# mahyarnajibi/SNIPER

Measured on AMD Instinct MI355X. Metric: train chips/sec (512x512, R101), higher is better.
Workload: dtype f16; 1 GPU; ResNet-101 Faster-RCNN SNIPER 3-scale, batch 20 x 512x512 fp16 per GPU (BASELINE configs[1]); step = GPU anchor labelling + fwd + bwd + grad all-reduce + SGD on HBM-resident chips (epoch chip generation / box assignment and image decode+resize are outside the step); f16 MFMA operands, f32 accumulation / losses / master weights; chips_per_gpu=20, global_batch=20, parallelism=dp1

## Files before the change

include/sniper_hip.h:

```cpp
#ifndef SNIPER_HIP_H
#define SNIPER_HIP_H

#include <stddef.h>
#include <stdint.h>

#ifdef __cplusplus
extern "C" {
#endif

typedef void *sn_stream_t;

enum { SN_OK = 0, SN_ERR_ARG = 1, SN_ERR_HIP = 2, SN_ERR_WORKSPACE = 3, SN_ERR_UNSUPPORTED = 4 };

int sn_version(void);
const char *sn_last_error(void);
int sn_debug_option(const char *name, int value);

int sn_iou_f64(const double *d_boxes, int N, const double *d_query, int K, double *d_out, int mode, sn_stream_t stream);

int sn_chips_num_candidates(int width, int height, int chipsize, int stride);
size_t sn_chips_workspace_bytes(int total_cand, int max_boxes_per_unit);
int sn_chips_generate_batch(const float *d_boxes, const int32_t *d_box_off, const int32_t *d_meta, const int32_t *d_perm,
                            const int32_t *d_cand_off, int U, int max_boxes_per_unit, void *d_mask_ws, float *d_out_chips,
                            int32_t *d_out_ids, int32_t *d_out_count, sn_stream_t stream);
// ... 55 lines not shown
                           int Cout, int out_pix_stride, int KH, int KW, int stride, int pad, int dil, int relu, void *ws,
                           size_t ws_bytes, sn_stream_t stream);
int sn_conv_fwd_dual_ok(int N, int H, int W, int Cin, int in_pix_stride, int Cout, int out_pix_stride, int res_pix_stride, int KH,
                        int KW, int stride, int pad, int dil, int y2_pix_stride);
int sn_conv_fwd_dual(const void *x, const void *w, const float *bias, const void *residual, void *y, int N, int H, int W, int Cin,
                     int in_pix_stride, int Cout, int out_pix_stride, int res_pix_stride, int KH, int KW, int stride, int pad, int dil,
                     int relu, void *y2, int y2_pix_stride, const float *y2_scale, const float *y2_shift, int y2_relu, void *ws,
                     size_t ws_bytes, sn_stream_t stream);
int sn_conv_tune(int cfg);

int sn_conv_fwd_stats_blocks(int N, int H, int W, int Cin, int in_pix_stride, int Cout, int out_pix_stride, int res_pix_stride,
                             int KH, int KW, int stride, int pad, int dil);
int sn_conv_fwd_stats(const void *x, const void *w, const float *bias, const void *residual, void *y, int N, int H, int W, int Cin,
                      int in_pix_stride, int Cout, int out_pix_stride, int res_pix_stride, int KH, int KW, int stride, int pad,
                      int dil, int relu, float *stats, sn_stream_t stream);
int sn_conv_stem_fwd(const void *xp, const void *w, const float *bias, void *y, int N, int Hp, int Wp, int Ho, int Wo, int Cout,
                     int out_pix_stride, int KH, int KWP, int stride, int relu, int out_f32, sn_stream_t stream);
size_t sn_conv_stem_wgrad_workspace_bytes(int N, int Ho, int Wo, int Cout, int KH, int KWP);
int sn_conv_stem_wgrad(const void *dy, const void *xp, float *dw, int N, int Hp, int Wp, int Ho, int Wo, int Cout, int dy_pix_stride,
                       int KH, int KWP, int stride, void *ws, size_t ws_bytes, sn_stream_t stream);
int sn_conv_dgrad(const void *dy, const void *wt, const void *accumulate, void *dx, int N, int H, int W, int Cin,
                  int dx_pix_stride, int Cout, int dy_pix_stride, int acc_pix_stride, int KH, int KW, int stride, int pad, int dil,
                  int out_f32, sn_stream_t stream);
int sn_conv_dgrad_by_class(int on);
int sn_conv_dgrad_bn_blocks(int N, int H, int W, int Cin, int dx_pix_stride, int Cout, int dy_pix_stride, int acc_pix_stride, int KH,
                            int KW, int stride, int pad, int dil);
int sn_conv_dgrad_bn(const void *dy, const void *wt, const void *accumulate, void *dx, int N, int H, int W, int Cin, int dx_pix_stride,
                     int Cout, int dy_pix_stride, int acc_pix_stride, int KH, int KW, int stride, int pad, int dil, const void *bn_x,
                     int bn_x_pix_stride, const float *bn_scale, const float *bn_shift, const float *bn_mean, int bn_act,
                     float *partials, sn_stream_t stream);
// ... 285 lines not shown
```

sniper_amd/csrc/conv.hip:

```cpp
#include <algorithm>
#include <atomic>

#include "conv_common.h"

#include <stdlib.h>

__device__ __forceinline__ int swz(int row, int chunk) { return chunk ^ ((0x78 >> (2 * ((row >> 2) & 3))) & 3); }

template <int BM, int BN, bool DGRAD>
__global__ __launch_bounds__(256) void conv_igemm_kernel(const ConvParams p) {
  constexpr int BK = 32;
  constexpr int WM = BM / 2, WN = BN / 2;
  constexpr int MI = WM / 16, NI = WN / 16;
  constexpr int AR = BM / 64, BR = BN / 64;
  __shared__ __attribute__((aligned(16))) half_t sA[2][BM * BK];
  __shared__ __attribute__((aligned(16))) half_t sB[2][BN * BK];

  const int tid = threadIdx.x, lane = tid & 63, wave = tid >> 6;
  const int wm = wave >> 1, wn = wave & 1;
  const int m0 = blockIdx.x * BM, n0 = blockIdx.y * BN;
  const int chunk = tid & 3, lrow = tid >> 2;

  int a_base[AR], a_h[AR], a_w[AR];
  bool a_ok[AR];
// ... 414 lines not shown
}

SN_EXPORT int sn_conv_fwd_stats(const void *x, const void *w, const float *bias, const void *residual, void *y, int N, int H, int W,
                                int Cin, int in_pix_stride, int Cout, int out_pix_stride, int res_pix_stride, int KH, int KW,
                                int stride, int pad, int dil, int relu, float *stats, sn_stream_t stream) {
  ConvParams p;
  conv_fwd_params(p, x, w, bias, residual, y, N, H, W, Cin, in_pix_stride, Cout, out_pix_stride, res_pix_stride, KH, KW, stride, pad,
                  dil, relu, 0);
  if (int rc = conv_check(p, "sn_conv_fwd_stats")) return rc;
  SN_REQUIRE(stats && Cout % 4 == 0 && out_pix_stride % 4 == 0 && (!residual || res_pix_stride % 4 == 0),
             "sn_conv_fwd_stats: statistics need 8-byte aligned output rows (query sn_conv_fwd_stats_blocks)");
  p.stats = stats;
  return conv_launch<false>(p, sn_stream(stream));
}

SN_EXPORT int sn_conv_stem_fwd(const void *xp, const void *w, const float *bias, void *y, int N, int Hp, int Wp, int Ho, int Wo,
                               int Cout, int out_pix_stride, int KH, int KWP, int stride, int relu, int out_f32,
                               sn_stream_t stream) {
  ConvParams p;
  p.x = (const half_t *)xp; p.w = (const half_t *)w; p.y = y; p.bias = bias; p.res = nullptr;
  p.N = N; p.H = Hp; p.W = Wp; p.Cin = 4 * KWP; p.in_ps = 4;
  p.Ho = Ho; p.Wo = Wo; p.Nout = Cout; p.out_ps = out_pix_stride; p.res_ps = 0;
  p.KH = KH; p.KW = 1; p.stride = stride; p.pad = 0; p.dil = 1;
  p.M = N * Ho * Wo; p.relu = relu; p.out_f32 = out_f32;
  SN_REQUIRE((Ho - 1) * stride + KH <= Hp && (Wo - 1) * stride + KWP <= Wp, "sn_conv_stem_fwd: padded input too small");
  SN_REQUIRE(stride % 2 == 0 && Wp % 2 == 0 && KWP % 2 == 0, "sn_conv_stem_fwd: 16-byte alignment needs even stride/pitch");
  if (int rc = conv_check(p, "sn_conv_stem_fwd")) return rc;
  return conv_launch<false>(p, sn_stream(stream));
}

// ... 375 lines not shown
```

sniper_amd/csrc/conv_common.h:

```cpp
#pragma once
#include <atomic>
#include "common.h"

struct ConvParams {
  const half_t *x;
  const half_t *w;
  void *y;
  const float *bias;
  const half_t *res;
  int N, H, W;
  int Cin, in_ps;
  int Ho, Wo;
  int Nout, out_ps, res_ps;
  int KH, KW, stride, pad, dil;
  int M;
  int relu, out_f32;
  unsigned x_bytes, w_bytes;
  const half_t *bn_x = nullptr;
  const float *bn_scale = nullptr, *bn_shift = nullptr, *bn_mean = nullptr;
  int bn_x_ps = 0, bn_act = 0;
  unsigned fda_mul = 1, fda_sh = 0, fdb_mul = 1, fdb_sh = 0;
  int rows_img = 1, row_len = 1;
  int cls = 0, cls_mc = 0;
  int ksplit = 1, ksplit_grid = 0;
  long ksplit_stride = 0;
  unsigned long long *trace = nullptr;
  half_t *out2 = nullptr;
  const float *o2_scale = nullptr, *o2_shift = nullptr;
  int out2_ps = 0, o2_relu = 0;
  int tiles_per_wg = 1;
  float *stats = nullptr;
};


static inline void conv_fastdiv_fill(ConvParams &p) {
  p.rows_img = p.cls ? (p.Ho / 2) * (p.Wo / 2) : p.Ho * p.Wo;
  p.row_len = p.cls ? p.Wo / 2 : p.Wo;
  const SnDiv a = sn_div_make((unsigned)p.rows_img), b = sn_div_make((unsigned)p.row_len);
  p.fda_mul = a.mul; p.fda_sh = a.sh;
  p.fdb_mul = b.mul; p.fdb_sh = b.sh;
}

typedef __attribute__((address_space(3))) void *lds_ptr_t;
typedef short short4v __attribute__((vector_size(8)));

__device__ __forceinline__ void dma16(__amdgpu_buffer_rsrc_t rsrc, half_t *dst, unsigned voff) {
// ... 13 lines not shown

struct ConvDmaConfig { int bm, bn, threads, stages, lds_bytes; };
constexpr int kConvPersistWgs = 512;
static inline int conv_persist_tiles_per_wg(int M, int Nout, int bm, int bn) {
  if (M % bm || Nout % bn) return 0;
  const long mt = M / bm, nt = Nout / bn, tiles = mt * nt;
  if (mt % 8 || tiles < 2 * kConvPersistWgs || tiles % kConvPersistWgs) return 0;
  return (int)(tiles / kConvPersistWgs);
}
constexpr int kConvDmaConfigs = 26;
ConvDmaConfig conv_dma_config(int cfg);
int conv_dma_launch(const ConvParams &p, bool dgrad, int cfg, hipStream_t s);
void conv_dma_set_trace(unsigned long long *buf);
int conv_dma_ragged_cfg(int cfg, bool dgrad);
int conv_dma_ragged_launch(const ConvParams &p, bool dgrad, int cfg, hipStream_t s);

struct WgradParams {
  const half_t *dy;
  const half_t *x;
  float *dw;
  int N, H, W, Ho, Wo, Cin, Cout, dy_ps, x_ps;
  int KH, KW, stride, pad, dil;
  int units_per_split;
  float *slab;
  size_t slab_stride;
  int gx, gy, gz, per_xcd;
};

__device__ __forceinline__ bool wgrad_block(const WgradParams &p, int &bx, int &by, int &bz) {
  const int b = blockIdx.x;
// ... 38 lines not shown
```

sniper_amd/csrc/conv_dma.hip:

```cpp
#include "conv_dma_kernel.h"

ConvDmaConfig conv_dma_config(int cfg) { return (cfg >= 1 && cfg <= kConvDmaConfigs) ? kCfg[cfg] : kCfg[0]; }

template <bool DGRAD>
static int launch_cfg(const ConvParams &p, int cfg, hipStream_t s) {
  switch (cfg) {
    case 4: launch_config<DGRAD, 4>(p, s); break;
    case 5: launch_config<DGRAD, 5>(p, s); break;
    case 6: launch_config<DGRAD, 6>(p, s); break;
    case 7: launch_config<DGRAD, 7>(p, s); break;
    case 14: launch_config<DGRAD, 14>(p, s); break;
    case 16: launch_config<DGRAD, 16>(p, s); break;
    case 18: launch_config<DGRAD, 18>(p, s); break;
    case 24: launch_config<DGRAD, 24>(p, s); break;
    case 26: launch_config<DGRAD, 26>(p, s); break;
    default: SN_REQUIRE(false, "conv_dma_launch: unknown configuration %d", cfg);
  }
  SN_CHECK_LAUNCH();
  return SN_OK;
}

static std::atomic<unsigned long long *> g_conv_trace{nullptr};
void conv_dma_set_trace(unsigned long long *buf) { g_conv_trace.store(buf, std::memory_order_relaxed); }

int conv_dma_launch(const ConvParams &p, bool dgrad, int cfg, hipStream_t s) {
  ConvParams q = p;
  q.trace = g_conv_trace.load(std::memory_order_relaxed);
  if (p.Cin % 64 != 0) return conv_dma_ragged_launch(q, dgrad, cfg, s);
  return dgrad ? launch_cfg<true>(q, cfg, s) : launch_cfg<false>(q, cfg, s);
}
```

sniper_amd/csrc/conv_dma_body.h:

```cpp
  constexpr int NW = WMW * WNW, T = 64 * (NW + (PS ? 4 : 0)), BK = 64;
  static_assert(!PERSIST || (!PS && S == 2), "the persistent tile loop is written for the two-stage unspecialised pipeline");
  static_assert(!PERSIST || !RAGGED, "the persistent tile loop walks whole 64-channel steps");
  constexpr int NL = PS ? 4 : NW;
  constexpr int WTM = BM / WMW, WTN = BN / WNW;
  constexpr int MI = WTM / 16, NI = WTN / 16;
  constexpr int PA = BM / 8, PB = BN / 8;
  constexpr int AGW = (PA + NL - 1) / NL, BGW = (PB + NL - 1) / NL;
  constexpr int L = AGW + BGW;
  constexpr int STAGE = (BM + BN) * BK;
  constexpr bool kPingPong = NW == 8 && S >= 3;
  static_assert(BM % 8 == 0 && BN % 8 == 0 && WTM % 16 == 0 && WTN % 16 == 0, "tile / wave shape");
  static_assert(PA >= NL * (AGW - 1) + 1 && PB >= NL * (BGW - 1) + 1 && (AGW == 1 ? PA >= NL : true) && (BGW == 1 ? PB >= NL : true),
                "a wave's repeated piece must exist");
  static_assert((S - 1) * L < 64, "vmcnt is a 6-bit counter");
  constexpr int RED = PERSIST ? WMW * 2 * BN * 2 : 0;
  constexpr bool kBnLds = PERSIST && DGRAD;
  constexpr int COEF = kBnLds ? 3 * 512 : 0;
  static_assert(!kBnLds || BN <= 128, "one LDS-DMA piece carries 128 coefficients");
  __shared__ __attribute__((aligned(1024))) half_t lds[S * STAGE + RED + COEF];

  constexpr bool kSplitOk = !PERSIST && !DGRAD && BM * BN <= 160 * 128;
  int kz = 0;
  int lin = blockIdx.x;
  if (kSplitOk && p.ksplit > 1) {
    kz = lin / p.ksplit_grid;
    lin -= kz * p.ksplit_grid;
  }
  auto tile_of = [&](int l, int &mt_, int &nt_) {
    const int xcd = l & 7, j = l >> 3;
    nt_ = j % ntiles;
    mt_ = (j / ntiles) * 8 + xcd;
  };
  int nt, mt;
  tile_of(lin, mt, nt);
// ... 41 lines not shown

  int a_base[AGW], a_h[AGW], a_w[AGW];
  bool a_ok[AGW];
  int a_grp[AGW], b_grp[BGW];
#pragma unroll
  for (int i = 0; i < AGW; ++i) a_grp[i] = (lw + NL * i < PA) ? lw + NL * i : lw + NL * (i - 1);
#pragma unroll
  for (int i = 0; i < BGW; ++i) b_grp[i] = (lw + NL * i < PB) ? lw + NL * i : lw + NL * (i - 1);
  unsigned a_voff[AGW];
  auto gather_rows = [&](int gm0) {
    if constexpr (PERSIST) {
#pragma unroll
      for (int i = 0; i < AGW; ++i) a_voff[i] = (unsigned)(gm0 + 8 * a_grp[i] + lrow) * ((unsigned)p.in_ps * 2u) + (unsigned)gchunk * 16u;
      return;
    }
#pragma unroll
    for (int i = 0; i < AGW; ++i) {
      const int m = gm0 + 8 * a_grp[i] + lrow;
      a_ok[i] = m < Mrows;
      int img, oy, ox;
      row_decompose(a_ok[i] ? m : 0, img, oy, ox);
      a_base[i] = img * p.H * p.W;
      if (DGRAD) { a_h[i] = oy + p.pad; a_w[i] = ox + p.pad; }
      else { a_h[i] = oy * p.stride - p.pad; a_w[i] = ox * p.stride - p.pad; }
    }
  };
  gather_rows(m0);
  const int taps = p.KH * p.KW;
  const int kpt = RAGGED ? (p.Cin + BK - 1) / BK : p.Cin / BK;
  const bool tail_in = !RAGGED || gchunk * 8 < p.Cin - (kpt - 1) * BK;
// ... 17 lines not shown
      const int r = 8 * b_grp[i] + lrow;
      const int n = gn0 + (r & ~31) + ((r & 15) >> 2) * 8 + ((r >> 4) & 1) * 4 + (r & 3);
      w_voff[i] = n < p.Nout ? (unsigned)n * wrow_bytes + (unsigned)gchunk * 16u : kOob;
      if constexpr (RAGGED) w_voff_l[i] = tail_in ? w_voff[i] : kOob;
    }
  };
  gather_cols(n0);
  int g_kh = kh0, g_kw = kw0, g_kc = 0;
  if (kSplitOk && t_begin > 0) {
    const int tap = t_begin / kpt;
    g_kc = t_begin - tap * kpt;
    g_kh = tap / p.KW;
    g_kw = tap - g_kh * p.KW;
  }
  auto tap_setup = [&]() {
    if constexpr (PERSIST) return;
#pragma unroll
    for (int i = 0; i < AGW; ++i) {
      int sy, sx;
      bool ok = a_ok[i];
      if (DGRAD) {
        const int ty = a_h[i] - g_kh * p.dil, tx = a_w[i] - g_kw * p.dil;
        if (p.stride == 1) { sy = ty; sx = tx; }
        else if (p.stride == 2) { sy = ty >> 1; sx = tx >> 1; ok = ok && !((ty | tx) & 1); }
        else { sy = ty / p.stride; sx = tx / p.stride; ok = ok && (sy * p.stride == ty) && (sx * p.stride == tx); }
        ok = ok && ty >= 0 && tx >= 0 && sy < p.H && sx < p.W;
      } else {
        sy = a_h[i] + g_kh * p.dil; sx = a_w[i] + g_kw * p.dil;
        ok = ok && (unsigned)sy < (unsigned)p.H && (unsigned)sx < (unsigned)p.W;
      }
      a_voff[i] = ok ? (unsigned)(a_base[i] + sy * p.W + sx) * in_ps_bytes + (unsigned)gchunk * 16u : kOob;
// ... 12 lines not shown
#pragma unroll
        for (int i = 0; i < AGW; ++i) dma16(rx, sa + a_grp[i] * 512, av[i]);
#pragma unroll
        for (int i = 0; i < BGW; ++i) dma16(rw, sb + b_grp[i] * 512, wv[i]);
      };
      if (g_kc == kpt - 1) pieces(a_voff_l, w_voff_l);
      else pieces(a_voff, w_voff);
    } else {
#pragma unroll
    for (int i = 0; i < AGW; ++i)
      dma16(rx, sa + a_grp[i] * 512, a_voff[i]);
#pragma unroll
    for (int i = 0; i < BGW; ++i)
      dma16(rw, sb + b_grp[i] * 512, w_voff[i]);
    }
    if constexpr (PERSIST) {
      ++g_kc;
    } else if (++g_kc == kpt) {
      g_kc = 0;
      g_kw += kstep;
      if (g_kw >= p.KW) { g_kw = kw0; g_kh += kstep; }
      tap_setup();
    }
  };

  auto fetch_seek = [&](int l, int step) {
    int fmt, fnt;
    tile_of(l, fmt, fnt);
    gather_rows(fmt * BM);
    gather_cols(fnt * BN);
    g_kc = step;
// ... 55 lines not shown
    } else {
      const int m = row_pixel(mr < Mrows ? mr : 0);
      return (mr < Mrows && n < p.Nout) ? *reinterpret_cast<const half8 *>(pre_src + (size_t)m * pre_ps + n) : half8{0, 0, 0, 0, 0, 0, 0, 0};
    }
  };
  auto pre_load_tile = [&](int pm0, int pn0) {
#pragma unroll
    for (int i = 0; i < MI; ++i)
#pragma unroll
      for (int jp = 0; jp < NP; ++jp) rpre[i][jp] = pre_load(pm0, pn0, i, jp);
  };
  if constexpr (kPre) if ((pre_res || pre_bnx) && !producer) pre_load_tile(m0, n0);

  if constexpr (PS) {
    if (producer) {
#pragma unroll
      for (int s = 0; s < S - 1; ++s)
        if (s < nk) issue(s);
      int nxt = S - 1;
      for (int t = 0; t < nk; ++t) {
        const int young = min(S - 2, nk - 1 - t);
        if (S > 3 && young >= 2) wait_vmcnt<(S > 3 ? 2 : 0) * L>();
        else if (S > 2 && young == 1) wait_vmcnt<(S > 2 ? 1 : 0) * L>();
        else wait_vmcnt<0>();
        __builtin_amdgcn_s_barrier();
        if (t + S - 1 < nk) issue(nxt);
        nxt = nxt + 1 == S ? 0 : nxt + 1;
      }
    } else {
      half8 fa0[MI], fb0[NI], fa1[MI], fb1[NI];
      auto read = [&](int buf, int ks, half8 (&fa)[MI], half8 (&fb)[NI]) {
        const half_t *const base = lds + buf * STAGE;
        const int co = (sw ^ (ks * 4)) * 8;
#pragma unroll
        for (int i = 0; i < MI; ++i) fa[i] = *reinterpret_cast<const half8 *>(base + a_rd + i * 16 * BK + co);
#pragma unroll
        for (int jn = 0; jn < NI; ++jn) fb[jn] = *reinterpret_cast<const half8 *>(base + b_rd + jn * 16 * BK + co);
      };
      auto mma = [&](const half8 (&fa)[MI], const half8 (&fb)[NI]) {
// ... 3 lines not shown
          for (int jn = 0; jn < NI; ++jn) acc[i][jn] = __builtin_amdgcn_mfma_f32_16x16x32_f16(fb[jn], fa[i], acc[i][jn], 0, 0, 0);
      };
      auto interleave = [&]() {
#pragma unroll
        for (int k = 0; k < MI + NI; ++k) {
          __builtin_amdgcn_sched_group_barrier(0x008, 2, 0);
          __builtin_amdgcn_sched_group_barrier(0x100, 1, 0);
        }
        __builtin_amdgcn_sched_group_barrier(0x008, MI * NI - 2 * (MI + NI) > 0 ? MI * NI - 2 * (MI + NI) : 0, 0);
        __builtin_amdgcn_sched_barrier(0);
      };
      auto step_barrier = [&]() {
        asm volatile("s_waitcnt lgkmcnt(0)" ::: "memory");
        __builtin_amdgcn_s_barrier();
      };
      if (nk > 0) {
        step_barrier();
        stamp(1);
        read(0, 0, fa0, fb0);
        __builtin_amdgcn_sched_barrier(0);
      }
      int cur = 0, nxt = 1;
      for (int t = 0; t + 1 < nk; ++t) {
        mma(fa0, fb0);
        read(cur, 1, fa1, fb1);
        interleave();
        step_barrier();
        __builtin_amdgcn_sched_barrier(0);
        mma(fa1, fb1);
        read(nxt, 0, fa0, fb0);
// ... 350 lines not shown
```

sniper_amd/csrc/conv_dma_kernel.h:

```cpp
#pragma once
#include "conv_common.h"
#include <type_traits>

template <int CTRL>
__device__ __forceinline__ float dpp_add(float v) {
  return v + __builtin_bit_cast(float, __builtin_amdgcn_update_dpp(0, __builtin_bit_cast(int, v), CTRL, 0xF, 0xF, false));
}
__device__ __forceinline__ float row16_sum(float v) {
  v = dpp_add<0xB1>(v);
  v = dpp_add<0x4E>(v);
  v = dpp_add<0x141>(v);
  return dpp_add<0x140>(v);
}

__device__ __forceinline__ half8 load16_untracked(const half_t *ptr) {
  floatx4 v;
  asm volatile("global_load_dwordx4 %0, %1, off" : "=v"(v) : "v"(ptr) : "memory");
  return __builtin_bit_cast(half8, v);
}
__device__ __forceinline__ floatx4 lds_read16_untracked(const void *ptr) {
  floatx4 v;
  const unsigned a = (unsigned)(unsigned long)(lds_ptr_t)const_cast<void *>(ptr);
  asm volatile("ds_read_b128 %0, %1" : "=v"(v) : "v"(a) : "memory");
  return v;
}
__device__ __forceinline__ void tie(floatx4 &v) { asm volatile("" : "+v"(v)); }
__device__ __forceinline__ void tie(half8 &x) {
  floatx4 v = __builtin_bit_cast(floatx4, x);
  asm volatile("" : "+v"(v));
  x = __builtin_bit_cast(half8, v);
}

template <bool DGRAD, int BM, int BN, int WMW, int WNW, int S, int MINW, bool PS = false, bool PERSIST = false>
__global__ __launch_bounds__(64 * (WMW * WNW + (PS ? 4 : 0)), MINW) void conv_dma_kernel(const ConvParams p, int mtiles, int ntiles) {
  constexpr bool RAGGED = false;
#include "conv_dma_body.h"
}
template <bool DGRAD, int BM, int BN, int WMW, int WNW, int S, int MINW, bool PS = false, bool PERSIST = false>
__global__ __launch_bounds__(64 * (WMW * WNW + (PS ? 4 : 0)), MINW) void conv_dma_ragged_kernel(const ConvParams p, int mtiles, int ntiles) {
  constexpr bool RAGGED = true;
#include "conv_dma_body.h"
}

template <bool DGRAD, int BM, int BN, int WMW, int WNW, int S, int MINW, bool PS = false, bool PERSIST = false, bool RAGGED = false>
static void launch_one(const ConvParams &p, hipStream_t s) {
  const int mtiles = (DGRAD && !PS && p.cls && BM * BN <= 160 * 128) ? 4 * sn_div_up(p.cls_mc, BM) : sn_div_up(p.M, BM), ntiles = sn_div_up(p.Nout, BN);
  const int base = sn_div_up(mtiles, 8) * 8 * ntiles;
  ConvParams q = p;
  q.ksplit_grid = base;
  if constexpr (PERSIST) {
    q.tiles_per_wg = conv_persist_tiles_per_wg(p.M, p.Nout, BM, BN);
    q.ksplit = 1;
    hipLaunchKernelGGL((conv_dma_kernel<DGRAD, BM, BN, WMW, WNW, S, MINW, PS, true>), dim3((unsigned)(base / q.tiles_per_wg)),
                       dim3(64 * WMW * WNW), 0, s, q, mtiles, ntiles);
  } else {
// ... 48 lines not shown
```

sniper_amd/csrc/nn_ops.hip:

```cpp
#include "common.h"
#include "softmax_grad.h"
#include <algorithm>

__global__ __launch_bounds__(256) void pack_stem_kernel(const float *__restrict__ x, half_t *__restrict__ out, int N, int C,
                                                        int H, int W, int Hp, int Wp, int pad_t, int pad_l,
                                                        const float *__restrict__ scale, const float *__restrict__ shift) {
  const long total = (long)N * Hp * Wp;
  for (long i = (long)blockIdx.x * blockDim.x + threadIdx.x; i < total; i += (long)gridDim.x * blockDim.x) {
    const int xp = (int)(i % Wp);
    const long t = i / Wp;
    const int yp = (int)(t % Hp), n = (int)(t / Hp);
    const int sy = yp - pad_t, sx = xp - pad_l;
    half_t v[4] = {0, 0, 0, 0};
    if ((unsigned)sy < (unsigned)H && (unsigned)sx < (unsigned)W) {
      for (int c = 0; c < C && c < 4; ++c) {
        float f = x[(((long)n * C + c) * H + sy) * W + sx];
        if (scale) f = f * scale[c] + shift[c];
        v[c] = (half_t)f;
      }
    }
    *reinterpret_cast<uint2 *>(out + i * 4) = *reinterpret_cast<uint2 *>(v);
  }
}

SN_EXPORT int sn_pack_stem_input(const float *x_nchw, void *out, int N, int C, int H, int W, int Hp, int Wp, int pad_t,
                                 int pad_l, const float *scale, const float *shift, sn_stream_t stream) {
  SN_REQUIRE(x_nchw && out && N > 0 && C >= 1 && C <= 4 && Hp >= H + pad_t && Wp >= W + pad_l,
             "sn_pack_stem_input: bad arguments");
  const long total = (long)N * Hp * Wp;
  hipLaunchKernelGGL(pack_stem_kernel, dim3(sn_blocks(total, 4096)), dim3(256), 0, sn_stream(stream), x_nchw, (half_t *)out, N, C, H, W,
                     Hp, Wp, pad_t, pad_l, scale, shift);
  SN_CHECK_LAUNCH();
  return SN_OK;
}

constexpr int kBnThreads = 256;
constexpr int kBnUnroll = 4;

__device__ __forceinline__ bool bn_act_pass(float y, int act) {
  return act == 0 || (act == 1 ? y > 0.f : (y >= 0.f && y <= 6.f));
}

__device__ __forceinline__ void bn_fwd_coefs(double mean, double var, float eps, float g, float beta, float &sc, float &sh, float &invstd) {
  invstd = (float)(1.0 / sqrt(var + (double)eps));
  sc = __fmul_rn(g, invstd);
  sh = __fmaf_rn(-__fmul_rn((float)mean, g), invstd, beta);
}
__device__ __forceinline__ float bn_running(float run, float stat, float momentum) {
  return __fmaf_rn(run, momentum, __fmul_rn(stat, 1.f - momentum));
}
__device__ __forceinline__ float bn_affine(float x, float sc, float sh) { return __fmaf_rn(x, sc, sh); }
__device__ __forceinline__ void bn_dx_coefs(float sc, float invstd, float mean, float dgamma, float dbeta, float invM, float &kb, float &kd) {
  const float t = __fmul_rn(__fmul_rn(invstd, dgamma), invM);
  kb = -__fmul_rn(sc, t);
  kd = __fmul_rn(sc, __fmaf_rn(mean, t, -__fmul_rn(dbeta, invM)));
}
__device__ __forceinline__ float bn_dx_value(float sc, float gf, float kb, float xf, float kd, float a) {
  return __fadd_rn(__fmaf_rn(sc, gf, __fmaf_rn(kb, xf, kd)), a);
}

struct BnMap {
  int cb, rpp, chunk, rl;
  bool on;
};
__device__ __forceinline__ BnMap bn_map(int C) {
  const int cpr = C >> 3;
// ... 148 lines not shown
  for (int c = threadIdx.x; c < d.C; c += 256) bn_global_channel(d.gamma, d.beta, d.mean, d.var, c, d.eps, d.scale, d.shift);
}

__global__ __launch_bounds__(256) void bn_apply_kernel(const half_t *__restrict__ x, half_t *__restrict__ y, int M, int C,
                                                       int ps_in, int ps_out, const float *__restrict__ scale,
                                                       const float *__restrict__ shift, int relu) {
  const int cpr = C >> 3;
  const long total = (long)M * cpr;
  for (long i = (long)blockIdx.x * blockDim.x + threadIdx.x; i < total; i += (long)gridDim.x * blockDim.x) {
    const int chunk = (int)(i % cpr);
    const long r = i / cpr;
    const half8 v = *reinterpret_cast<const half8 *>(x + r * ps_in + chunk * 8);
    half8 o;
#pragma unroll
    for (int j = 0; j < 8; ++j) {
      float f = bn_affine((float)v[j], scale[chunk * 8 + j], shift[chunk * 8 + j]);
      if (relu) f = f > 0.f ? f : 0.f;
      if (relu == 2) f = f < 6.f ? f : 6.f;
      o[j] = (half_t)f;
    }
    *reinterpret_cast<half8 *>(y + r * ps_out + chunk * 8) = o;
  }
}

__global__ __launch_bounds__(kBnThreads) void bn_bwd_reduce_kernel(const half_t *__restrict__ dy, const half_t *__restrict__ x,
                                                                   int M, int C, int ps_dy, int ps_x, int rows_per_block,
                                                                   const float *__restrict__ scale,
                                                                   const float *__restrict__ shift,
                                                                   const float *__restrict__ mean,
                                                                   int relu, float *__restrict__ part) {
  const BnMap m = bn_map(C);
  const int r0 = blockIdx.x * rows_per_block, r1 = min(M, r0 + rows_per_block);
  float s[8], q[8];
#pragma unroll
// ... 1358 lines not shown
```

sniper_amd/engine/ops.py:

```python
import os

import numpy as np
import torch

from .. import hip
from ..mx.symbol import _bool, _tup
from .executor import F16, F32, Val, _pad8
from .shapes import slot_inputs

REGISTRY = {}


def register(*names):
    def deco(cls):
        for n in names:
            REGISTRY[n] = cls
        return cls
    return deco


class Step(object):
    def __init__(self, ex, node, wants_f32):
        self.ex, self.node, self.wants_f32 = ex, node, wants_f32
        self.a = node.attrs
# ... 116 lines not shown
            self.y = self.new_out('act', alloc=False)
            self.y.t = self.x.t
        else:
            self.y = self.new_out('act')
        self.y.needs_grad = ex.for_training and (self.x.needs_grad or self.gamma.trainable or self.beta.trainable) \
            and not self.is_stem
        chain = cons
        if self.act and len(cons) == 1:
            chain = ex.consumers.get((id(cons[0]), 0), [])
        self.sole_consumer = chain[0] if len(chain) == 1 else None
        self.stats_from = None
        if ex.for_training and not self.global_stats and not self.is_stem and self.x.fmt == 'act':
            conv = _conv_behind(self.x)
            if conv is not None:
                self.stats_from = conv.request_stats()

    def batched_refresh(self):
        return self.ex.for_training and self.global_stats and (self.gamma.trainable or self.beta.trainable)

    def fold_global(self):
        hip.call('sn_bn_global_scale_shift', None if self.fix_gamma else self.gamma.master, self.beta.master, self.mean, self.var,
                 self.C, self.eps, self.scale, self.shift, hip.stream())
        self._global_ready = True

    def params_changed(self, only_trainable=False):
        if self.batched_refresh():
            self._global_ready = True
            return
        if not (only_trainable and self.global_stats and not self.gamma.trainable and not self.beta.trainable):
            self._global_ready = False
# ... 23 lines not shown
            return
        g = None if self.fix_gamma else self.gamma.master
        if not self._use_batch_stats():
            if not self._global_ready:
                self.fold_global()
            if self.is_stem:
                return
        if self.is_stem:
            raise NotImplementedError('batch-statistics BatchNorm on the raw image input')
        x = ex.as_act(self.x)
        n, h, w, c = self.x.nhwc()
        M = n * h * w
        if self._use_batch_stats():
            if self.bws is None:
                self.bws = ex.empty((hip.query('sn_bn_workspace_bytes', M, c),), torch.uint8)
            if self.stats_from is not None:
                part, nblk = self.stats_from
                hip.call('sn_bn_apply_blocks', part, nblk, x, self.y.t, M, c, c, c, self.eps, self.momentum, g, self.beta.master,
                         self.mean, self.var, self.scale, self.shift, self.save_mean, self.save_invstd, self.act, hip.stream())
                return
            else:
                hip.call('sn_bn_stats', x, M, c, c, self.bws, hip.stream())
                hip.call('sn_bn_finalize', self.bws, M, c, self.eps, self.momentum, g, self.beta.master, self.mean,
                         self.var, self.scale, self.shift, self.save_mean, self.save_invstd, hip.stream())
        hip.call('sn_bn_apply', x, self.y.t, M, c, c, c, self.scale, self.shift, self.act, hip.stream())

    def backward(self):
        ex = self.ex
        if self.y.grad is None or not self.y.needs_grad:
            return
# ... 187 lines not shown
        if self.x.needs_grad:
            dx, acc = ex.input_grad_dst(self.x)
            self.launch_dgrad(dy, Op, acc, dx)
            ex.input_grad_done(self.x, dx)
        self.y.grad = None


@register('Convolution')
class ConvolutionStep(_GemmLike):
    def setup(self):
        self.fused_residual = self.fused_dst = None
        self.fold_bn = None
        self.dual_bn = None
        self.stats_buf, self.stats_blocks = None, 0
        self.bnb_buf = None
        _GemmLike.setup(self)

    def setup_geom(self):
        a = self.a
        self.k = _tup(a['kernel'])
        self.s = _tup(a.get('stride', (1, 1)))
        self.p = _tup(a.get('pad', (0, 0)))
        self.d = _tup(a.get('dilate', (1, 1)))
        assert self.s[0] == self.s[1] and self.p[0] == self.p[1] and self.d[0] == self.d[1], 'square geometry only'
        self.N, self.C, self.H, self.W = self.x.shape
        _, self.O, self.Ho, self.Wo = self.out_shape()
        g = int(a.get('num_group', 1))
        if g < 1 or self.C % g or self.O % g:
            raise ValueError('%s: num_group=%d does not divide %d -> %d channels' % (self.node.name, g, self.C, self.O))
        self.groups = g
        self.depthwise = g > 1 and g == self.C == self.O
# ... 68 lines not shown

    def _fwd_depthwise(self, x, dst, bias):
        if bias is not None or self.out_f32:
            raise NotImplementedError('depthwise convolution with bias / fp32 output (%s)' % self.node.name)
        hip.call('sn_dwconv_fwd', x, self.w.w16, dst, self.N, self.H, self.W, self.C, self.C, self.O, self.k[0], self.k[1],
                 self.s[0], self.p[0], self.d[0], hip.stream())

    def _fwd_igemm(self, x, dst, bias):
        ex, geom = self.ex, self.geom()
        res = None
        if self.fused_residual is not None:
            res, dst = self.fused_residual.t, self.fused_dst.t
        if self.stats_buf is not None and ex.is_train:
            if self._stats_blocks() != self.stats_blocks:
                raise RuntimeError('%s: kernel selection changed after the statistics buffer was sized' % self.node.name)
            hip.call('sn_conv_fwd_stats', x, self.w.w16, bias, res, dst, *geom, 0, self.stats_buf, hip.stream())
            return
        w, b, relu = self._fwd_operands(bias)
        if not ex.for_training and not self.out_f32:
            if self._splitk_bytes is None:
                self._splitk_bytes = int(hip.query('sn_conv_fwd_splitk_workspace_bytes', *geom))
            ws = ex.ws.get(self._splitk_bytes) if self._splitk_bytes else None
            dual = self.dual_bn
            if dual is not None and not ex.is_train:
                if not dual._global_ready:
                    dual.fold_global()
                hip.call('sn_conv_fwd_dual', x, w, b, res, dst, *geom, relu, dual.y.t, self.O, dual.scale, dual.shift,
                         1 if dual.act == 1 else 0, ws, self._splitk_bytes, hip.stream())
                return
            if self._splitk_bytes:
# ... 877 lines not shown
```

Baseline: 994.6 chips/s.

## Fuse preceding BatchNorm apply into 1x1 conv forward staging waves during training

When a training-mode BatchNorm feeds only a 1x1 stride-1 conv whose plan selects the specialised DMA config, the conv kernel's producer waves now apply the BN affine and ReLU to the raw input tiles in LDS. They also write the normalised activation out for the backward pass. The BN step then computes only its statistics and coefficients, which removes a separate elementwise read/write pass over the activation. The cost is extra LDS traffic and producer-wave work inside the conv pipeline, plus one more barrier. Eligibility is narrow (a single config, Cin up to 2048), and the path can be turned off with an environment variable.

```diff
diff --git a/include/sniper_hip.h b/include/sniper_hip.h
--- a/include/sniper_hip.h
+++ b/include/sniper_hip.h
@@ -93,6 +93,12 @@
 int sn_conv_fwd_stats(const void *x, const void *w, const float *bias, const void *residual, void *y, int N, int H, int W, int Cin,
                       int in_pix_stride, int Cout, int out_pix_stride, int res_pix_stride, int KH, int KW, int stride, int pad,
                       int dil, int relu, float *stats, sn_stream_t stream);
+int sn_conv_fwd_stats_bnin_ok(int N, int H, int W, int Cin, int in_pix_stride, int Cout, int out_pix_stride, int res_pix_stride,
+                              int KH, int KW, int stride, int pad, int dil);
+int sn_conv_fwd_stats_bnin(const void *x, const void *w, const float *bias, const void *residual, void *y, int N, int H, int W, int Cin,
+                           int in_pix_stride, int Cout, int out_pix_stride, int res_pix_stride, int KH, int KW, int stride, int pad,
+                           int dil, int relu, float *stats, const float *bn_scale, const float *bn_shift, int bn_act, void *a_out,
+                           int a_out_pix_stride, sn_stream_t stream);
 int sn_conv_stem_fwd(const void *xp, const void *w, const float *bias, void *y, int N, int Hp, int Wp, int Ho, int Wo, int Cout,
                      int out_pix_stride, int KH, int KWP, int stride, int relu, int out_f32, sn_stream_t stream);
 size_t sn_conv_stem_wgrad_workspace_bytes(int N, int Ho, int Wo, int Cout, int KH, int KWP);
diff --git a/sniper_amd/csrc/bn_math.h b/sniper_amd/csrc/bn_math.h
--- /dev/null
+++ b/sniper_amd/csrc/bn_math.h
@@ -0,0 +1,18 @@
+#pragma once
+#include "common.h"
+
+__device__ __forceinline__ bool bn_act_pass(float y, int act) {
+  return act == 0 || (act == 1 ? y > 0.f : (y >= 0.f && y <= 6.f));
+}
+__device__ __forceinline__ float bn_affine(float x, float sc, float sh) { return __fmaf_rn(x, sc, sh); }
+__device__ __forceinline__ float bn_apply_value(float x, float sc, float sh, int act) {
+  float f = bn_affine(x, sc, sh);
+  if (act) f = f > 0.f ? f : 0.f;
+  if (act == 2) f = f < 6.f ? f : 6.f;
+  return f;
+}
+__device__ __forceinline__ half_t bn_apply_f16(float x, float sc, float sh, int act) {
+  float f = bn_apply_value(x, sc, sh, act);
+  asm("" : "+v"(f));
+  return (half_t)f;
+}
diff --git a/sniper_amd/csrc/conv.hip b/sniper_amd/csrc/conv.hip
--- a/sniper_amd/csrc/conv.hip
+++ b/sniper_amd/csrc/conv.hip
@@ -452,6 +452,51 @@
   return conv_launch<false>(p, sn_stream(stream));
 }
 
+static bool conv_bnin_geom_ok(const ConvParams &p) {
+  return p.KH == 1 && p.KW == 1 && p.stride == 1 && p.pad == 0 && p.dil == 1 && p.Cin % 64 == 0 && p.Cin <= kConvBninMaxCin &&
+         p.in_ps % 8 == 0 && p.Ho > 0 && p.Wo > 0 && p.Nout % 4 == 0 && p.out_ps % 4 == 0 && p.res_ps % 4 == 0;
+}
+
+SN_EXPORT int sn_conv_fwd_stats_bnin_ok(int N, int H, int W, int Cin, int in_pix_stride, int Cout, int out_pix_stride, int res_pix_stride,
+                                        int KH, int KW, int stride, int pad, int dil) {
+  ConvParams p;
+  conv_fwd_params(p, nullptr, nullptr, nullptr, nullptr, nullptr, N, H, W, Cin, in_pix_stride, Cout, out_pix_stride, res_pix_stride, KH,
+                  KW, stride, pad, dil, 0, 0);
+  if (N <= 0 || H <= 0 || W <= 0 || Cin <= 0 || Cout <= 0 || KH <= 0 || KW <= 0 || stride <= 0 || dil <= 0 || pad < 0) return 0;
+  if (!conv_bnin_geom_ok(p)) return 0;
+  if ((long)p.N * p.H * p.W * p.in_ps >= (1l << 31) || (long)p.M * p.out_ps >= (1l << 31)) return 0;
+  if (conv_plan(p, false).dma != kConvBninCfg) return 0;
+  return conv_dma_choice_balanced(p.M, p.Nout, p.Cin / 64, false) == kConvBninCfg ? 1 : 0;
+}
+
+SN_EXPORT int sn_conv_fwd_stats_bnin(const void *x, const void *w, const float *bias, const void *residual, void *y, int N, int H, int W,
+                                     int Cin, int in_pix_stride, int Cout, int out_pix_stride, int res_pix_stride, int KH, int KW,
+                                     int stride, int pad, int dil, int relu, float *stats, const float *bn_scale, const float *bn_shift,
+                                     int bn_act, void *a_out, int a_out_pix_stride, sn_stream_t stream) {
+  ConvParams p;
+  conv_fwd_params(p, x, w, bias, residual, y, N, H, W, Cin, in_pix_stride, Cout, out_pix_stride, res_pix_stride, KH, KW, stride, pad,
+                  dil, relu, 0);
+  if (int rc = conv_check(p, "sn_conv_fwd_stats_bnin")) return rc;
+  SN_REQUIRE(stats && Cout % 4 == 0 && out_pix_stride % 4 == 0 && (!residual || res_pix_stride % 4 == 0),
+             "sn_conv_fwd_stats_bnin: statistics need 8-byte aligned output rows");
+  SN_REQUIRE(bn_scale && bn_shift && a_out, "sn_conv_fwd_stats_bnin: null BatchNorm pointer");
+  SN_REQUIRE(bn_act == 0 || bn_act == 1, "sn_conv_fwd_stats_bnin: bn_act must be 0 (none) or 1 (ReLU), got %d", bn_act);
+  SN_REQUIRE(KH == 1 && KW == 1 && stride == 1 && pad == 0 && dil == 1, "sn_conv_fwd_stats_bnin: the layer must be 1 x 1, stride 1, unpadded");
+  SN_REQUIRE(Cin % 64 == 0 && Cin <= kConvBninMaxCin, "sn_conv_fwd_stats_bnin: Cin must be a multiple of 64 and <= %d (got %d)",
+             kConvBninMaxCin, Cin);
+  SN_REQUIRE(a_out_pix_stride >= Cin && a_out_pix_stride % 8 == 0, "sn_conv_fwd_stats_bnin: a_out rows must be 16-byte addressable (pitch %d)",
+             a_out_pix_stride);
+  SN_REQUIRE((long)p.M * a_out_pix_stride < (1l << 31), "sn_conv_fwd_stats_bnin: a_out too large for 32-bit offsets");
+  SN_REQUIRE(a_out != x, "sn_conv_fwd_stats_bnin: a_out must not alias x (every column tile reads the raw input)");
+  p.stats = stats;
+  p.bnin_scale = bn_scale; p.bnin_shift = bn_shift; p.bnin_act = bn_act;
+  p.bnin_out = (half_t *)a_out; p.bnin_out_ps = a_out_pix_stride;
+  const ConvPlan pl = conv_plan(p, false);
+  SN_REQUIRE(pl.dma == kConvBninCfg, "sn_conv_fwd_stats_bnin: the layer's plan is configuration %d, not %d (query sn_conv_fwd_stats_bnin_ok)",
+             pl.dma, kConvBninCfg);
+  return conv_launch<false>(p, sn_stream(stream));
+}
+
 SN_EXPORT int sn_conv_stem_fwd(const void *xp, const void *w, const float *bias, void *y, int N, int Hp, int Wp, int Ho, int Wo,
                                int Cout, int out_pix_stride, int KH, int KWP, int stride, int relu, int out_f32,
                                sn_stream_t stream) {
diff --git a/sniper_amd/csrc/conv_common.h b/sniper_amd/csrc/conv_common.h
--- a/sniper_amd/csrc/conv_common.h
+++ b/sniper_amd/csrc/conv_common.h
@@ -30,6 +30,9 @@
   int out2_ps = 0, o2_relu = 0;
   int tiles_per_wg = 1;
   float *stats = nullptr;
+  const float *bnin_scale = nullptr, *bnin_shift = nullptr;
+  half_t *bnin_out = nullptr;
+  int bnin_out_ps = 0, bnin_act = 0;
 };
 
 
@@ -73,6 +76,9 @@
 void conv_dma_set_trace(unsigned long long *buf);
 int conv_dma_ragged_cfg(int cfg, bool dgrad);
 int conv_dma_ragged_launch(const ConvParams &p, bool dgrad, int cfg, hipStream_t s);
+constexpr int kConvBninCfg = 18;
+constexpr int kConvBninMaxCin = 2048;
+int conv_dma_bnin_launch(const ConvParams &p, int cfg, hipStream_t s);
 
 struct WgradParams {
   const half_t *dy;
diff --git a/sniper_amd/csrc/conv_dma.hip b/sniper_amd/csrc/conv_dma.hip
--- a/sniper_amd/csrc/conv_dma.hip
+++ b/sniper_amd/csrc/conv_dma.hip
@@ -26,6 +26,10 @@
 int conv_dma_launch(const ConvParams &p, bool dgrad, int cfg, hipStream_t s) {
   ConvParams q = p;
   q.trace = g_conv_trace.load(std::memory_order_relaxed);
+  if (p.bnin_scale) {
+    SN_REQUIRE(!dgrad, "conv_dma_launch: an input BatchNorm rides on forward launches only");
+    return conv_dma_bnin_launch(q, cfg, s);
+  }
   if (p.Cin % 64 != 0) return conv_dma_ragged_launch(q, dgrad, cfg, s);
   return dgrad ? launch_cfg<true>(q, cfg, s) : launch_cfg<false>(q, cfg, s);
 }
diff --git a/sniper_amd/csrc/conv_dma_bnin.hip b/sniper_amd/csrc/conv_dma_bnin.hip
--- /dev/null
+++ b/sniper_amd/csrc/conv_dma_bnin.hip
@@ -0,0 +1,20 @@
+#include "conv_dma_kernel.h"
+
+int conv_dma_bnin_launch(const ConvParams &p, int cfg, hipStream_t s) {
+  SN_REQUIRE(cfg == kConvBninCfg, "conv_dma_bnin_launch: configuration %d is not instantiated", cfg);
+  constexpr int BM = 160, BN = 128, WMW = 2, WNW = 2, S = 4;
+  static_assert(kCfg[kConvBninCfg].bm == BM && kCfg[kConvBninCfg].bn == BN && kCfg[kConvBninCfg].threads == 64 * (WMW * WNW + 4) &&
+                    kCfg[kConvBninCfg].stages == S && kCfg[kConvBninCfg].lds_bytes == S * (BM + BN) * 128,
+                "kCfg and the template arguments of the BNIN instantiation disagree");
+  static_assert(kCfg[kConvBninCfg].lds_bytes + 2 * kConvBninMaxCin * 4 <= 160 * 1024, "ring + coefficient table exceed the LDS");
+  SN_REQUIRE(p.bnin_scale && p.bnin_shift && p.bnin_out && p.ksplit <= 1 && p.cls == 0 && p.Cin % 64 == 0 && p.Cin <= kConvBninMaxCin &&
+                 p.KH == 1 && p.KW == 1 && p.stride == 1 && p.pad == 0,
+             "conv_dma_bnin_launch: not a whole-tap 1 x 1 forward launch with an input BatchNorm");
+  const int mtiles = sn_div_up(p.M, BM), ntiles = sn_div_up(p.Nout, BN);
+  ConvParams q = p;
+  q.ksplit_grid = sn_div_up(mtiles, 8) * 8 * ntiles;
+  hipLaunchKernelGGL((conv_dma_bnin_kernel<BM, BN, WMW, WNW, S, 1>), dim3((unsigned)q.ksplit_grid), dim3(64 * (WMW * WNW + 4)), 0, s, q, mtiles,
+                     ntiles);
+  SN_CHECK_LAUNCH();
+  return SN_OK;
+}
diff --git a/sniper_amd/csrc/conv_dma_body.h b/sniper_amd/csrc/conv_dma_body.h
--- a/sniper_amd/csrc/conv_dma_body.h
+++ b/sniper_amd/csrc/conv_dma_body.h
@@ -17,7 +17,9 @@
   constexpr bool kBnLds = PERSIST && DGRAD;
   constexpr int COEF = kBnLds ? 3 * 512 : 0;
   static_assert(!kBnLds || BN <= 128, "one LDS-DMA piece carries 128 coefficients");
-  __shared__ __attribute__((aligned(1024))) half_t lds[S * STAGE + RED + COEF];
+  static_assert(!BNIN || (PS && !PERSIST && !DGRAD && !RAGGED && PA % NL == 0), "the input BatchNorm rides on the specialised forward kernel's staging waves");
+  constexpr int BNTAB = BNIN ? 2 * kConvBninMaxCin * 2 : 0;
+  __shared__ __attribute__((aligned(1024))) half_t lds[S * STAGE + RED + COEF + BNTAB];
 
   constexpr bool kSplitOk = !PERSIST && !DGRAD && BM * BN <= 160 * 128;
   int kz = 0;
@@ -89,6 +91,14 @@
       for (int i = 0; i < AGW; ++i) a_voff[i] = (unsigned)(gm0 + 8 * a_grp[i] + lrow) * ((unsigned)p.in_ps * 2u) + (unsigned)gchunk * 16u;
       return;
     }
+    if constexpr (BNIN) {
+#pragma unroll
+      for (int i = 0; i < AGW; ++i) {
+        const int m = gm0 + 8 * a_grp[i] + lrow;
+        a_voff[i] = m < Mrows ? (unsigned)m * ((unsigned)p.in_ps * 2u) + (unsigned)gchunk * 16u : 0xFFFFFF00u;
+      }
+      return;
+    }
 #pragma unroll
     for (int i = 0; i < AGW; ++i) {
       const int m = gm0 + 8 * a_grp[i] + lrow;
@@ -136,7 +146,7 @@
     g_kw = tap - g_kh * p.KW;
   }
   auto tap_setup = [&]() {
-    if constexpr (PERSIST) return;
+    if constexpr (PERSIST || BNIN) return;
 #pragma unroll
     for (int i = 0; i < AGW; ++i) {
       int sy, sx;
@@ -179,7 +189,7 @@
     for (int i = 0; i < BGW; ++i)
       dma16(rw, sb + b_grp[i] * 512, w_voff[i]);
     }
-    if constexpr (PERSIST) {
+    if constexpr (PERSIST || BNIN) {
       ++g_kc;
     } else if (++g_kc == kpt) {
       g_kc = 0;
@@ -265,15 +275,72 @@
 
   if constexpr (PS) {
     if (producer) {
+      [[maybe_unused]] unsigned v_stage = 0, v_piece = 0, v_tab = 0, v_ok = 0, v_rows = 0;
+      [[maybe_unused]] int v_act = 0;
+      [[maybe_unused]] char *v_out = nullptr;
+      if constexpr (BNIN) {
+        float *const bntab = reinterpret_cast<float *>(lds + S * STAGE + RED + COEF);
+        const __amdgpu_buffer_rsrc_t rs = __builtin_amdgcn_make_buffer_rsrc(const_cast<float *>(p.bnin_scale), 0, p.Cin * 4, 0x00020000);
+        const __amdgpu_buffer_rsrc_t rh = __builtin_amdgcn_make_buffer_rsrc(const_cast<float *>(p.bnin_shift), 0, p.Cin * 4, 0x00020000);
+#pragma unroll
+        for (int j = 0; j < 2; ++j) {
+          const int pc = lw + NL * j;
+          dma16(rs, reinterpret_cast<half_t *>(bntab + pc * 256), (unsigned)(pc * 1024 + lane * 16));
+          dma16(rh, reinterpret_cast<half_t *>(bntab + kConvBninMaxCin + pc * 256), (unsigned)(pc * 1024 + lane * 16));
+        }
+        v_piece = lds_addr(lds) + (unsigned)(lw * 1024 + lane * 16);
+        v_tab = lds_addr(bntab) + (unsigned)gchunk * 32u;
+        v_out = reinterpret_cast<char *>(p.bnin_out) + ((size_t)(m0 + 8 * lw + lrow) * p.bnin_out_ps + gchunk * 8) * 2;
+        v_rows = (unsigned)(8 * NL * p.bnin_out_ps) * 2u;
+#pragma unroll
+        for (int i = 0; i < AGW; ++i)
+          if (nt == 0 && a_voff[i] != kOob) v_ok |= 1u << i;
+        v_act = p.bnin_act;
+        keep_in_vgpr(v_stage); keep_in_vgpr(v_piece); keep_in_vgpr(v_tab); keep_in_vgpr(v_ok); keep_in_vgpr(v_rows); keep_in_vgpr(v_act);
+        keep_in_vgpr(v_out);
+      }
 #pragma unroll
       for (int s = 0; s < S - 1; ++s)
         if (s < nk) issue(s);
+      if constexpr (BNIN) {
+        const int pro = min(S - 1, nk);
+        if (S > 3 && pro >= 3) wait_vmcnt<(S > 3 ? 3 : 0) * L>();
+        else if (S > 2 && pro == 2) wait_vmcnt<(S > 2 ? 2 : 0) * L>();
+        else wait_vmcnt<L>();
+        __builtin_amdgcn_s_barrier();
+      }
       int nxt = S - 1;
       for (int t = 0; t < nk; ++t) {
         const int young = min(S - 2, nk - 1 - t);
         if (S > 3 && young >= 2) wait_vmcnt<(S > 3 ? 2 : 0) * L>();
         else if (S > 2 && young == 1) wait_vmcnt<(S > 2 ? 1 : 0) * L>();
         else wait_vmcnt<0>();
+        if constexpr (BNIN) {
+          const unsigned a = v_piece + v_stage;
+          floatx4 cf[4], xv[AGW];
+          cf[0] = lds_read16_at<0>(v_tab);
+          cf[1] = lds_read16_at<16>(v_tab);
+          cf[2] = lds_read16_at<kConvBninMaxCin * 4>(v_tab);
+          cf[3] = lds_read16_at<kConvBninMaxCin * 4 + 16>(v_tab);
+          static_for([&](auto i) { xv[i] = lds_read16_at<i * NL * 1024>(a); }, std::make_integer_sequence<int, AGW>{});
+          asm volatile("s_waitcnt lgkmcnt(0)" ::: "memory");
+#pragma unroll
+          for (int k4 = 0; k4 < 4; ++k4) tie(cf[k4]);
+#pragma unroll
+          for (int i = 0; i < AGW; ++i) tie(xv[i]);
+          static_for([&](auto i) {
+            const half8 xh = __builtin_bit_cast(half8, xv[i]);
+            half8 o;
+#pragma unroll
+            for (int r = 0; r < 8; ++r) o[r] = bn_apply_f16((float)xh[r], cf[r >> 2][r & 3], cf[2 + (r >> 2)][r & 3], v_act & 1);
+            lds_write16_at<i * NL * 1024>(a, __builtin_bit_cast(floatx4, o));
+            if (v_ok & (1u << i)) global_store16(v_out + (size_t)i * v_rows, o);
+          }, std::make_integer_sequence<int, AGW>{});
+          asm volatile("s_waitcnt lgkmcnt(0)" ::: "memory");
+          v_tab += BK * 4;
+          v_out += BK * 2;
+          v_stage = v_stage + STAGE * 2 == S * STAGE * 2 ? 0u : v_stage + STAGE * 2;
+        }
         __builtin_amdgcn_s_barrier();
         if (t + S - 1 < nk) issue(nxt);
         nxt = nxt + 1 == S ? 0 : nxt + 1;
@@ -307,6 +374,7 @@
         asm volatile("s_waitcnt lgkmcnt(0)" ::: "memory");
         __builtin_amdgcn_s_barrier();
       };
+      if constexpr (BNIN) __builtin_amdgcn_s_barrier();
       if (nk > 0) {
         step_barrier();
         stamp(1);
diff --git a/sniper_amd/csrc/conv_dma_kernel.h b/sniper_amd/csrc/conv_dma_kernel.h
--- a/sniper_amd/csrc/conv_dma_kernel.h
+++ b/sniper_amd/csrc/conv_dma_kernel.h
@@ -1,6 +1,8 @@
 #pragma once
 #include "conv_common.h"
+#include "bn_math.h"
 #include <type_traits>
+#include <utility>
 
 template <int CTRL>
 __device__ __forceinline__ float dpp_add(float v) {
@@ -24,6 +26,25 @@
   asm volatile("ds_read_b128 %0, %1" : "=v"(v) : "v"(a) : "memory");
   return v;
 }
+__device__ __forceinline__ unsigned lds_addr(const void *ptr) { return (unsigned)(unsigned long)(lds_ptr_t)const_cast<void *>(ptr); }
+template <int OFF>
+__device__ __forceinline__ floatx4 lds_read16_at(unsigned a) {
+  floatx4 v;
+  asm volatile("ds_read_b128 %0, %1 offset:%2" : "=v"(v) : "v"(a), "n"(OFF) : "memory");
+  return v;
+}
+template <int OFF>
+__device__ __forceinline__ void lds_write16_at(unsigned a, floatx4 v) {
+  asm volatile("ds_write_b128 %0, %1 offset:%2" ::"v"(a), "v"(v), "n"(OFF) : "memory");
+}
+__device__ __forceinline__ void global_store16(char *ptr, half8 v) {
+  typedef __attribute__((address_space(1))) half8 *gptr_t;
+  *(gptr_t)ptr = v;
+}
+template <class V>
+__device__ __forceinline__ void keep_in_vgpr(V &x) { asm volatile("" : "+v"(x)); }
+template <class F, int... I>
+__device__ __forceinline__ void static_for(F &&f, std::integer_sequence<int, I...>) { (f(std::integral_constant<int, I>{}), ...); }
 __device__ __forceinline__ void tie(floatx4 &v) { asm volatile("" : "+v"(v)); }
 __device__ __forceinline__ void tie(half8 &x) {
   floatx4 v = __builtin_bit_cast(floatx4, x);
@@ -33,12 +54,17 @@
 
 template <bool DGRAD, int BM, int BN, int WMW, int WNW, int S, int MINW, bool PS = false, bool PERSIST = false>
 __global__ __launch_bounds__(64 * (WMW * WNW + (PS ? 4 : 0)), MINW) void conv_dma_kernel(const ConvParams p, int mtiles, int ntiles) {
-  constexpr bool RAGGED = false;
+  constexpr bool RAGGED = false, BNIN = false;
 #include "conv_dma_body.h"
 }
 template <bool DGRAD, int BM, int BN, int WMW, int WNW, int S, int MINW, bool PS = false, bool PERSIST = false>
 __global__ __launch_bounds__(64 * (WMW * WNW + (PS ? 4 : 0)), MINW) void conv_dma_ragged_kernel(const ConvParams p, int mtiles, int ntiles) {
-  constexpr bool RAGGED = true;
+  constexpr bool RAGGED = true, BNIN = false;
+#include "conv_dma_body.h"
+}
+template <int BM, int BN, int WMW, int WNW, int S, int MINW>
+__global__ __launch_bounds__(64 * (WMW * WNW + 4), MINW) void conv_dma_bnin_kernel(const ConvParams p, int mtiles, int ntiles) {
+  constexpr bool DGRAD = false, PS = true, PERSIST = false, RAGGED = false, BNIN = true;
 #include "conv_dma_body.h"
 }
 
diff --git a/sniper_amd/csrc/nn_ops.hip b/sniper_amd/csrc/nn_ops.hip
--- a/sniper_amd/csrc/nn_ops.hip
+++ b/sniper_amd/csrc/nn_ops.hip
@@ -1,4 +1,5 @@
 #include "common.h"
+#include "bn_math.h"
 #include "softmax_grad.h"
 #include <algorithm>
 
@@ -37,9 +38,6 @@
 constexpr int kBnThreads = 256;
 constexpr int kBnUnroll = 4;
 
-__device__ __forceinline__ bool bn_act_pass(float y, int act) {
-  return act == 0 || (act == 1 ? y > 0.f : (y >= 0.f && y <= 6.f));
-}
 
 __device__ __forceinline__ void bn_fwd_coefs(double mean, double var, float eps, float g, float beta, float &sc, float &sh, float &invstd) {
   invstd = (float)(1.0 / sqrt(var + (double)eps));
@@ -49,7 +47,6 @@
 __device__ __forceinline__ float bn_running(float run, float stat, float momentum) {
   return __fmaf_rn(run, momentum, __fmul_rn(stat, 1.f - momentum));
 }
-__device__ __forceinline__ float bn_affine(float x, float sc, float sh) { return __fmaf_rn(x, sc, sh); }
 __device__ __forceinline__ void bn_dx_coefs(float sc, float invstd, float mean, float dgamma, float dbeta, float invM, float &kb, float &kd) {
   const float t = __fmul_rn(__fmul_rn(invstd, dgamma), invM);
   kb = -__fmul_rn(sc, t);
@@ -228,10 +225,7 @@
     half8 o;
 #pragma unroll
     for (int j = 0; j < 8; ++j) {
-      float f = bn_affine((float)v[j], scale[chunk * 8 + j], shift[chunk * 8 + j]);
-      if (relu) f = f > 0.f ? f : 0.f;
-      if (relu == 2) f = f < 6.f ? f : 6.f;
-      o[j] = (half_t)f;
+      o[j] = bn_apply_f16((float)v[j], scale[chunk * 8 + j], shift[chunk * 8 + j], relu);
     }
     *reinterpret_cast<half8 *>(y + r * ps_out + chunk * 8) = o;
   }
diff --git a/sniper_amd/engine/ops.py b/sniper_amd/engine/ops.py
--- a/sniper_amd/engine/ops.py
+++ b/sniper_amd/engine/ops.py
@@ -154,6 +154,7 @@
             conv = _conv_behind(self.x)
             if conv is not None:
                 self.stats_from = conv.request_stats()
+        self.absorbed_by = None
 
     def batched_refresh(self):
         return self.ex.for_training and self.global_stats and (self.gamma.trainable or self.beta.trainable)
@@ -207,6 +208,16 @@
         if self._use_batch_stats():
             if self.bws is None:
                 self.bws = ex.empty((hip.query('sn_bn_workspace_bytes', M, c),), torch.uint8)
+            if self.absorbed_by is not None and self.absorbed_by.bn_in_active():
+                if self.stats_from is not None:
+                    part, nblk = self.stats_from
+                    hip.call('sn_bn_finalize_blocks', part, nblk, M, c, self.eps, self.momentum, g, self.beta.master, self.mean, self.var,
+                             self.scale, self.shift, self.save_mean, self.save_invstd, hip.stream())
+                else:
+                    hip.call('sn_bn_stats', x, M, c, c, self.bws, hip.stream())
+                    hip.call('sn_bn_finalize', self.bws, M, c, self.eps, self.momentum, g, self.beta.master, self.mean,
+                             self.var, self.scale, self.shift, self.save_mean, self.save_invstd, hip.stream())
+                return
             if self.stats_from is not None:
                 part, nblk = self.stats_from
                 hip.call('sn_bn_apply_blocks', part, nblk, x, self.y.t, M, c, c, c, self.eps, self.momentum, g, self.beta.master,
@@ -424,7 +435,28 @@
         self.dual_bn = None
         self.stats_buf, self.stats_blocks = None, 0
         self.bnb_buf = None
+        self.bn_in = None
         _GemmLike.setup(self)
+        self._claim_bn_in()
+
+    def _claim_bn_in(self):
+        ex = self.ex
+        if not ex.for_training or os.environ.get('SNIPER_TRAIN_BN_IN', '1') == '0':
+            return
+        if self.is_stem or self.groups > 1 or self.out_f32 or self.x.fmt != 'act':
+            return
+        bn = self.x.producer
+        if not isinstance(bn, BatchNormStep) or bn.global_stats or bn.is_stem or bn.folded_into is not None or bn.x.fmt != 'act':
+            return
+        if bn.act not in (0, 1) or bn.sole_consumer is not self.node or bn.absorbed_by is not None:
+            return
+        if not hip.query('sn_conv_fwd_stats_bnin_ok', *self.geom()):
+            return
+        self.bn_in = bn
+        bn.absorbed_by = self
+
+    def bn_in_active(self):
+        return self.bn_in is not None and self.stats_buf is not None and self.ex.is_train
 
     def setup_geom(self):
         a = self.a
@@ -523,6 +555,11 @@
         if self.stats_buf is not None and ex.is_train:
             if self._stats_blocks() != self.stats_blocks:
                 raise RuntimeError('%s: kernel selection changed after the statistics buffer was sized' % self.node.name)
+            if self.bn_in_active():
+                bn = self.bn_in
+                hip.call('sn_conv_fwd_stats_bnin', ex.as_act(bn.x), self.w.w16, bias, res, dst, *geom, 0, self.stats_buf, bn.scale,
+                         bn.shift, bn.act, x, self.C, hip.stream())
+                return
             hip.call('sn_conv_fwd_stats', x, self.w.w16, bias, res, dst, *geom, 0, self.stats_buf, hip.stream())
             return
         w, b, relu = self._fwd_operands(bias)
```

Result: no change. 1001 chips/s (median of 6 runs) (+0.6%).
